# halismai/bpvo

Hardware: AMD Instinct MI355X
Metric: GN iterations/s (1241x376 bit-planes 8ch, 4 levels, Tukey; linearise + solve + update = 1, the reference's _num_fun_evals) (higher is better)
Workload: dtype f32 (+f64 projection/interpolation)

## Files before the change

bpvo_amd/csrc/kernels_frame.hip:

```cpp
#include <algorithm>
#include <cstdlib>

#include "frame_common.h"

namespace bpvo_hip {

__device__ __forceinline__ const FrameJob& level_job(const FrameJob* jobs, unsigned z, int nframes, int job_pitch)
{
  const unsigned lvl = z / (unsigned) nframes;
  return jobs[(size_t) lvl * job_pitch + (z - lvl * (unsigned) nframes)];
}

__global__ __launch_bounds__(256) void ingest_kernel(const FrameJob* jobs, const uint8_t* images, const float* disps, size_t npix, int skip_odd_disp)
{
  const FrameJob& j = jobs[blockIdx.z];
  const uint8_t* __restrict__ si = images + (size_t) blockIdx.z * npix;
  const float* __restrict__ sd = disps + (size_t) (skip_odd_disp == 2 ? blockIdx.z / 2 : blockIdx.z) * npix;
  uint8_t* __restrict__ di = const_cast<uint8_t*>(j.img.get());
  float* __restrict__ dd = const_cast<float*>(j.disp.get());
  const size_t t = (size_t) blockIdx.x * 256 + threadIdx.x, stride = (size_t) gridDim.x * 256;
  const bool w4 = (npix % 4 == 0) && (((uintptr_t) si | (uintptr_t) di) % 4 == 0);
  if(w4) {
    const uint32_t* s4 = reinterpret_cast<const uint32_t*>(si);
    uint32_t* d4 = reinterpret_cast<uint32_t*>(di);
    for(size_t k = t; k < npix / 4; k += stride) d4[k] = s4[k];
  } else {
    for(size_t k = t; k < npix; k += stride) di[k] = si[k];
  }
  if(skip_odd_disp && (blockIdx.z & 1)) return;
  const bool f4 = (npix % 4 == 0) && (((uintptr_t) sd | (uintptr_t) dd) % 16 == 0);
  if(f4) {
    const float4* s4 = reinterpret_cast<const float4*>(sd);
    float4* d4 = reinterpret_cast<float4*>(dd);
    for(size_t k = t; k < npix / 4; k += stride) d4[k] = load_stream(s4 + k);
  } else {
    for(size_t k = t; k < npix; k += stride) dd[k] = sd[k];
  }
}

constexpr int PDT_W = 64, PDT_H = 16;
constexpr int PDS_W = 2 * PDT_W + 3, PDS_H = 2 * PDT_H + 3;
constexpr int PDS_DW = (PDS_W + 3 + 3) / 4;
constexpr int PDS_PITCH = 4 * (PDS_DW + 2);
constexpr int PD_STACK = 4;
constexpr int PD_NPRE = (PDS_H * PDS_DW + 255) / 256;
__global__ __launch_bounds__(256) void pyrdown_u8_lds_kernel(const FrameJob* src_jobs, const FrameJob* dst_jobs)
{
  __shared__ __attribute__((aligned(16))) uint8_t s_src[PDS_H][PDS_PITCH];
  __shared__ __attribute__((aligned(8))) uint16_t s_h[PDS_H][PDT_W];
  __shared__ int s_off[PDS_H];
  const FrameJob& sj = src_jobs[blockIdx.z];
  const FrameJob& dj = dst_jobs[blockIdx.z];
  const int sw = sj.cols, sh = sj.rows, dw = dj.cols, dh = dj.rows;
  const int dx0 = blockIdx.x * PDT_W;
  const int lane = threadIdx.x & 63, wave = threadIdx.x >> 6;
  const uint8_t* __restrict__ s = sj.img;
  uint8_t* __restrict__ const d = const_cast<uint8_t*>(dj.img.get());
  const int c_first = 2 * dx0 - 2;
  const bool fast = c_first >= 3 && c_first + PDS_W + 3 <= sw;
  auto row_ptr = [&](int dy0, int r) { return s + (size_t) reflect101(min(2 * dy0 - 2 + r, sh + 1), sh) * sw + c_first; };
  uint32_t pre[PD_NPRE];
  auto prefetch = [&](int dy0) {
#pragma unroll
    for(int k = 0; k < PD_NPRE; ++k) {
      const int i = min((int) threadIdx.x + k * 256, PDS_H * PDS_DW - 1);
      const int r = i / PDS_DW, l = i - r * PDS_DW;
      const uintptr_t a = reinterpret_cast<uintptr_t>(row_ptr(dy0, r));
      const unsigned ll = min((unsigned) l, ((unsigned) (a & 3u) + PDS_W - 1) / 4u);
      pre[k] = *reinterpret_cast<const uint32_t*>(a - (a & 3u) + 4u * ll);
    }
  };
  const int dy_first = blockIdx.y * (PDT_H * PD_STACK);
  if(fast) prefetch(dy_first);
  for(int t = 0; t < PD_STACK; ++t) {
    const int dy0 = dy_first + t * PDT_H;
    if(dy0 >= dh) break;
    if(fast) {
#pragma unroll
      for(int k = 0; k < PD_NPRE; ++k) {
        const int i = (int) threadIdx.x + k * 256;
        if(i < PDS_H * PDS_DW) { const int r = i / PDS_DW, l = i - r * PDS_DW; reinterpret_cast<uint32_t*>(&s_src[r][0])[l] = pre[k]; }
      }
      if(t + 1 < PD_STACK && dy0 + PDT_H < dh) prefetch(dy0 + PDT_H);
    } else {
      for(int r = wave; r < PDS_H; r += 4) {
        const uint8_t* row = s + (size_t) reflect101(min(2 * dy0 - 2 + r, sh + 1), sh) * sw;
#pragma unroll
        for(int c0 = 0; c0 < PDS_W; c0 += 64) {
          const int c = c0 + lane;
          if(c < PDS_W) s_src[r][c] = row[reflect101(min(c_first + c, sw + 1), sw)];
        }
      }
    }
    if(threadIdx.x < PDS_H) s_off[threadIdx.x] = fast ? (int) (reinterpret_cast<uintptr_t>(row_ptr(dy0, threadIdx.x)) & 3u) : 0;
    __syncthreads();
    for(int idx = threadIdx.x; idx < PDS_H * (PDT_W / 4); idx += 256) {
      const int r = idx >> 4, xq = idx & 15;
      const uint2* q = reinterpret_cast<const uint2*>(&s_src[r][8 * xq]);
      const uint2 lo = q[0], hi = q[1];
      const unsigned off = (unsigned) s_off[r];
      const unsigned d0 = __builtin_amdgcn_alignbyte(lo.y, lo.x, off), d1 = __builtin_amdgcn_alignbyte(hi.x, lo.y, off),
                     d2 = __builtin_amdgcn_alignbyte(hi.y, hi.x, off);
      const unsigned kW = 0x04060401u;
      const unsigned h0 = __builtin_amdgcn_udot4(d0, kW, d1 & 0xffu, false);
      const unsigned h1 = __builtin_amdgcn_udot4(__builtin_amdgcn_alignbyte(d1, d0, 2), kW, (d1 >> 16) & 0xffu, false);
      const unsigned h2 = __builtin_amdgcn_udot4(d1, kW, d2 & 0xffu, false);
      const unsigned h3 = __builtin_amdgcn_udot4(__builtin_amdgcn_alignbyte(d2, d1, 2), kW, (d2 >> 16) & 0xffu, false);
      *reinterpret_cast<uint2*>(&s_h[r][4 * xq]) = make_uint2(h0 | (h1 << 16), h2 | (h3 << 16));
    }
    __syncthreads();
    const int ty = threadIdx.x >> 4, xq = threadIdx.x & 15;
    const int y = dy0 + ty, x = dx0 + 4 * xq;
    if(y < dh && x < dw) {
      unsigned v[4];
      uint2 tt[5];
#pragma unroll
      for(int k = 0; k < 5; ++k) tt[k] = *reinterpret_cast<const uint2*>(&s_h[2 * ty + k][4 * xq]);
#pragma unroll
      for(int e = 0; e < 4; ++e) {
        unsigned a[5];
#pragma unroll
        for(int k = 0; k < 5; ++k) { const unsigned w = (e < 2) ? tt[k].x : tt[k].y; a[k] = (e & 1) ? (w >> 16) : (w & 0xffffu); }
        v[e] = (a[0] + 4u * a[1] + 6u * a[2] + 4u * a[3] + a[4] + 128u) >> 8;
      }
      uint8_t* o = d + (size_t) y * dw + x;
      if(x + 3 < dw) {
        typedef uint32_t __attribute__((aligned(1))) u32_unaligned;
        *reinterpret_cast<u32_unaligned*>(o) = v[0] | (v[1] << 8) | (v[2] << 16) | (v[3] << 24);
      } else {
        for(int e = 0; e < 4 && x + e < dw; ++e) o[e] = (uint8_t) v[e];
      }
    }
    __syncthreads();
  }
}

constexpr int PA_T = 8;
constexpr int pa_edge(int steps) { return steps == 0 ? PA_T : 2 * pa_edge(steps - 1) + 3; }
template <int NL>
__global__ __launch_bounds__(256) void pyramid_levels_kernel(const FrameJob* jobs , int job_pitch)
{
  constexpr int E0 = pa_edge(NL), E1 = pa_edge(NL - 1);
  __shared__ uint8_t s_a[E0 * E0];
  __shared__ uint8_t s_b[E1 * E1];
  __shared__ uint16_t s_h[E0 * E1];
  int W[NL + 1], H[NL + 1], xlo[NL + 1], xhi[NL + 1], ylo[NL + 1], yhi[NL + 1];
#pragma unroll
  for(int k = 0; k <= NL; ++k) { const FrameJob& j = jobs[(size_t) k * job_pitch + blockIdx.z]; W[k] = j.cols; H[k] = j.rows; }
  xlo[NL] = blockIdx.x * PA_T; xhi[NL] = min(xlo[NL] + PA_T, W[NL]) - 1;
  ylo[NL] = blockIdx.y * PA_T; yhi[NL] = min(ylo[NL] + PA_T, H[NL]) - 1;
#pragma unroll
  for(int k = NL - 1; k >= 0; --k) {
    xlo[k] = max(0, 2 * xlo[k + 1] - 2); xhi[k] = min(W[k] - 1, 2 * xhi[k + 1] + 2);
    ylo[k] = max(0, 2 * ylo[k + 1] - 2); yhi[k] = min(H[k] - 1, 2 * yhi[k + 1] + 2);
  }
  const int tid = threadIdx.x;
  {
    const uint8_t* __restrict__ src = jobs[blockIdx.z].img;
    const int nx = xhi[0] - xlo[0] + 1, ny = yhi[0] - ylo[0] + 1;
    for(int i = tid; i < nx * ny; i += 256) {
      const int r = i / nx, c = i - r * nx;
      s_a[r * E0 + c] = src[(size_t) (ylo[0] + r) * W[0] + xlo[0] + c];
    }
  }
  __syncthreads();
  uint8_t* cur = s_a;
  uint8_t* nxt = s_b;
  int pc = E0, pn = E1;
#pragma unroll
  for(int k = 0; k < NL; ++k) {
    const int snx = xhi[k] - xlo[k] + 1, sny = yhi[k] - ylo[k] + 1;
    const int dnx = xhi[k + 1] - xlo[k + 1] + 1, dny = yhi[k + 1] - ylo[k + 1] + 1;
    (void) snx;
    for(int i = tid; i < sny * dnx; i += 256) {
      const int r = i / dnx, c = i - r * dnx;
      const int x2 = 2 * (xlo[k + 1] + c);
      const uint8_t* row = cur + r * pc - xlo[k];
      const unsigned a0 = row[reflect101(x2 - 2, W[k])], a1 = row[reflect101(x2 - 1, W[k])], a2 = row[x2], a3 = row[reflect101(x2 + 1, W[k])],
                     a4 = row[reflect101(x2 + 2, W[k])];
      s_h[r * E1 + c] = (uint16_t) (a0 + 4u * a1 + 6u * a2 + 4u * a3 + a4);
    }
    __syncthreads();
    const int sh = NL - (k + 1);
    const int ox0 = (blockIdx.x * PA_T) << sh, ox1 = min(((blockIdx.x + 1) * PA_T) << sh, W[k + 1]);
    const int oy0 = (blockIdx.y * PA_T) << sh, oy1 = min(((blockIdx.y + 1) * PA_T) << sh, H[k + 1]);
    uint8_t* __restrict__ dst = const_cast<uint8_t*>(jobs[(size_t) (k + 1) * job_pitch + blockIdx.z].img.get());
    for(int i = tid; i < dny * dnx; i += 256) {
      const int r = i / dnx, c = i - r * dnx;
      const int y = ylo[k + 1] + r, x = xlo[k + 1] + c, y2 = 2 * y;
      const uint16_t* col = s_h + c - ylo[k] * E1;
      const unsigned b0 = col[reflect101(y2 - 2, H[k]) * E1], b1 = col[reflect101(y2 - 1, H[k]) * E1], b2 = col[y2 * E1],
                     b3 = col[reflect101(y2 + 1, H[k]) * E1], b4 = col[reflect101(y2 + 2, H[k]) * E1];
      const uint8_t v = (uint8_t) ((b0 + 4u * b1 + 6u * b2 + 4u * b3 + b4 + 128u) >> 8);
      nxt[r * pn + c] = v;
      if(x >= ox0 && x < ox1 && y >= oy0 && y < oy1) dst[(size_t) y * W[k + 1] + x] = v;
    }
    __syncthreads();
    { uint8_t* t = cur; cur = nxt; nxt = t; }
    { const int t = pc; pc = pn; pn = t; }
  }
}
void launch_pyramid_levels(hipStream_t s, const FrameJob* src_row, int job_pitch, int steps, int dW, int dR, int nframes)
{
  const dim3 grid((dW + PA_T - 1) / PA_T, (dR + PA_T - 1) / PA_T, nframes);
  if(steps == 3) hipLaunchKernelGGL(pyramid_levels_kernel<3>, grid, dim3(256), 0, s, src_row, job_pitch);
  else if(steps == 2) hipLaunchKernelGGL(pyramid_levels_kernel<2>, grid, dim3(256), 0, s, src_row, job_pitch);
  else hipLaunchKernelGGL(pyramid_levels_kernel<1>, grid, dim3(256), 0, s, src_row, job_pitch);
}

__global__ __launch_bounds__(256) void intensity_kernel(const FrameJob* jobs, int nframes, int job_pitch)
{
  const FrameJob& j = level_job(jobs, blockIdx.z, nframes, job_pitch);
  const int n = j.rows * j.cols;
  const int i = (blockIdx.x * 256 + threadIdx.x) * 4;
  if(i >= n) return;
  if(i + 3 < n && ((uintptr_t) (j.img + i) & 3) == 0) {
    const uchar4 v = *reinterpret_cast<const uchar4*>(j.img + i);
    *reinterpret_cast<float4*>(j.desc + i) = make_float4((float) v.x, (float) v.y, (float) v.z, (float) v.w);
  } else {
    for(int k = i; k < n && k < i + 4; ++k) j.desc[k] = (float) j.img[k];
  }
}

constexpr int ROWS_PER_THREAD = 4;
constexpr int CENSUS_ROWS = 8;
__global__ __launch_bounds__(256) void census_kernel(const FrameJob* jobs)
{
  const FrameJob& j = jobs[blockIdx.z];
  const int x = blockIdx.x * 64 + (threadIdx.x & 63);
  const int y0 = (blockIdx.y * 4 + (threadIdx.x >> 6)) * CENSUS_ROWS;
  const int W = j.cols, R = j.rows;
  if(x >= W || y0 >= R) return;
  const bool xin = x > 0 && x < W - 1;
  const int xm = max(x - 1, 0), xp = min(x + 1, W - 1);
  uint8_t w[CENSUS_ROWS + 2][3];
#pragma unroll
  for(int k = 0; k < CENSUS_ROWS + 2; ++k) {
    const uint8_t* p = j.img + (size_t) min(max(y0 - 1 + k, 0), R - 1) * W;
    w[k][0] = p[xm]; w[k][1] = p[x]; w[k][2] = p[xp];
  }
#pragma unroll
  for(int k = 0; k < CENSUS_ROWS; ++k) {
    const int y = y0 + k;
    if(y < R) {
      uint8_t out = 0;
      if(xin && y > 0 && y < R - 1) {
        const uint8_t ctr = w[k + 1][1];
        out = (uint8_t) (((w[k][0] >= ctr) << 0) | ((w[k][1] >= ctr) << 1) | ((w[k][2] >= ctr) << 2) | ((w[k + 1][0] >= ctr) << 3) |
                         ((w[k + 1][2] >= ctr) << 4) | ((w[k + 2][0] >= ctr) << 5) | ((w[k + 2][1] >= ctr) << 6) | ((w[k + 2][2] >= ctr) << 7));
      }
      j.cen[(size_t) y * W + x] = out;
    }
  }
}

constexpr int CB_TW = 64, CB_TH = 4;
__global__ __launch_bounds__(256) void census_blur_kernel(const FrameJob* jobs, int kc, int ks, int nframes, int job_pitch)
{
  __shared__ uint8_t s_src[(CB_TH + 4) * (CB_TW + 4)];
  __shared__ int s_tmp[(CB_TH + 4) * (CB_TW + 2)];
  __shared__ uint8_t s_b[(CB_TH + 2) * (CB_TW + 2)];
  const FrameJob& j = level_job(jobs, blockIdx.z, nframes, job_pitch);
  const int W = j.cols, R = j.rows;
  const int x0 = blockIdx.x * CB_TW, y0 = blockIdx.y * CB_TH;
  if(x0 >= W || y0 >= R) return;
  const int tid = threadIdx.x;
  for(int i = tid; i < (CB_TH + 4) * (CB_TW + 4); i += 256) {
    const int ly = i / (CB_TW + 4), lx = i - ly * (CB_TW + 4);
    const int gy = reflect101(min(y0 + ly - 2, R + 1), R), gx = reflect101(min(x0 + lx - 2, W + 1), W);
    s_src[i] = j.img[(size_t) gy * W + gx];
  }
  __syncthreads();
  for(int i = tid; i < (CB_TH + 4) * (CB_TW + 2); i += 256) {
    const int ly = i / (CB_TW + 2), lx = i - ly * (CB_TW + 2);
    const uint8_t* p = s_src + ly * (CB_TW + 4) + lx + 1;
    s_tmp[i] = (int) p[0] * kc + ((int) p[-1] + (int) p[1]) * ks;
  }
  __syncthreads();
  for(int i = tid; i < (CB_TH + 2) * (CB_TW + 2); i += 256) {
    const int ly = i / (CB_TW + 2), lx = i - ly * (CB_TW + 2);
    const int* t = s_tmp + (ly + 1) * (CB_TW + 2) + lx;
    const int v = (t[0] * kc + (t[-(CB_TW + 2)] + t[CB_TW + 2]) * ks + (1 << 15)) >> 16;
    s_b[i] = (uint8_t) min(255, max(0, v));
  }
  __syncthreads();
  const int lx = tid & 63, ly = tid >> 6;
  const int x = x0 + lx, y = y0 + ly;
  if(x >= W || y >= R) return;
  uint8_t out = 0;
  if(x > 0 && x < W - 1 && y > 0 && y < R - 1) {
    constexpr int P = CB_TW + 2;
    const uint8_t* p = s_b + (ly + 1) * P + lx + 1;
    const uint8_t c = p[0];
    out = (uint8_t) (((p[-P - 1] >= c) << 0) | ((p[-P] >= c) << 1) | ((p[-P + 1] >= c) << 2) | ((p[-1] >= c) << 3) |
                     ((p[1] >= c) << 4) | ((p[P - 1] >= c) << 5) | ((p[P] >= c) << 6) | ((p[P + 1] >= c) << 7));
  }
  j.cen[(size_t) y * W + x] = out;
}

#ifndef BP_TW_VALUE
#define BP_TW_VALUE 64
#define BP_TH_VALUE 8
#endif
constexpr int BP_TW = BP_TW_VALUE, BP_TH = BP_TH_VALUE, BP_HALO = 2;
constexpr int BP_PLANE = (BP_TH + 2 * BP_HALO) * BP_TW + 8;
__device__ __forceinline__ uint2 spread_planes(unsigned c)
{
  unsigned lo = c & 0xFu, hi = (c >> 4) & 0xFu;
  lo = (lo | (lo << 14)) & 0x00030003u; lo = (lo | (lo << 7)) & 0x01010101u;
  hi = (hi | (hi << 14)) & 0x00030003u; hi = (hi | (hi << 7)) & 0x01010101u;
  return make_uint2(lo, hi);
}

template <bool FROM_IMAGE>
__global__ __launch_bounds__(256) void bitplanes_blur_kernel(const FrameJob* jobs, float k0, float k1, float k2, int stack, int nframes, int job_pitch)
{
  constexpr int CR = BP_TH + 2 * BP_HALO, CC = BP_TW + 2 * BP_HALO;
  constexpr int CW = CC + 4;
  constexpr int IR = CR + 2, IC = CC + 2, IW = IC + 2;
  constexpr int NSRC = FROM_IMAGE ? IR * IC : CR * CC;
  constexpr int NPRE = (NSRC + 255) / 256;
  __shared__ uint2 s_cen[CR * CW];
  __shared__ uint8_t s_img[FROM_IMAGE ? IR * IW : 4];
  __shared__ float s_row[(BP_PLANE + CR * BP_TW) * 4];
  __shared__ float s_lut[18];
  const FrameJob& j = level_job(jobs, blockIdx.z, nframes, job_pitch);
  const int W = j.cols, R = j.rows;
  const int x0 = blockIdx.x * BP_TW;
  if(x0 >= W || (int) blockIdx.y * BP_TH * stack >= R) return;
  const int tid = threadIdx.x;
  const uint8_t* __restrict__ cen = FROM_IMAGE ? j.img : j.cen;
  float* __restrict__ const desc = j.desc;
  float* __restrict__ const ch0 = j.ch0;
  const bool lazy_level = FROM_IMAGE && j.lazy != 0;
  const bool lazy = lazy_level && x0 + BP_TW + 8 <= (W & ~3) && !(x0 == 0 && (W & 3) == 0);
  uint8_t* __restrict__ const cen_out = j.cen;
  if(tid < 18) {
    const float S0 = (float) (tid / 9), A = (float) (tid % 3), B = (float) ((tid / 3) % 3);
    s_lut[tid] = S0 * k0 + A * k1 + B * k2;
  }

  uint8_t pre[NPRE];
  auto prefetch = [&](int y0) {
#pragma unroll
    for(int k = 0; k < NPRE; ++k) {
      const int i = min(tid + k * 256, NSRC - 1);
      if constexpr(FROM_IMAGE) {
        const int ly = i / IC, lx = i - ly * IC;
        const int gy = min(max(y0 + ly - BP_HALO - 1, 0), R - 1), gx = min(max(x0 + lx - BP_HALO - 1, 0), W - 1);
        pre[k] = cen[(size_t) gy * W + gx];
      } else {
        const int ly = i / CC, lx = i - ly * CC;
        const int gy = reflect101(min(y0 + ly - BP_HALO, R + 1), R), gx = reflect101(min(x0 + lx - BP_HALO, W + 1), W);
        pre[k] = cen[(size_t) gy * W + gx];
      }
    }
  };
  auto stage = [&]() {
#pragma unroll
    for(int k = 0; k < NPRE; ++k) {
      const int i = tid + k * 256;
      if constexpr(FROM_IMAGE) {
        if(i < IR * IC) { const int ly = i / IC, lx = i - ly * IC; s_img[ly * IW + lx] = pre[k]; }
      } else {
        if(i < CR * CC) { const int ly = i / CC, lx = i - ly * CC; s_cen[ly * CW + lx] = spread_planes(pre[k]); }
      }
    }
  };
  const int ybase = blockIdx.y * BP_TH * stack;
  prefetch(ybase);
  stage();
  __syncthreads();
  for(int t = 0; t < stack; ++t) {
    const int y0 = ybase + t * BP_TH;
    if(y0 >= R) break;
    if constexpr(FROM_IMAGE) {
      for(int i = tid; i < CR * CC; i += 256) {
        const int ly = i / CC, lx = i - ly * CC;
        const int gy = reflect101(min(y0 + ly - BP_HALO, R + 1), R), gx = reflect101(min(x0 + lx - BP_HALO, W + 1), W);
        uint8_t out = 0;
        if(gx > 0 && gx < W - 1 && gy > 0 && gy < R - 1) {
          const uint8_t* p = s_img + (gy - (y0 - BP_HALO - 1)) * IW + (gx - (x0 - BP_HALO - 1));
          const uint8_t c = p[0];
          out = (uint8_t) (((p[-IW - 1] >= c) << 0) | ((p[-IW] >= c) << 1) | ((p[-IW + 1] >= c) << 2) | ((p[-1] >= c) << 3) |
                           ((p[1] >= c) << 4) | ((p[IW - 1] >= c) << 5) | ((p[IW] >= c) << 6) | ((p[IW + 1] >= c) << 7));
        }
        s_cen[ly * CW + lx] = spread_planes(out);
        if(lazy_level && ly >= BP_HALO && ly < BP_HALO + BP_TH && lx >= BP_HALO && lx < BP_HALO + BP_TW && y0 + ly - BP_HALO < R && x0 + lx - BP_HALO < W)
          cen_out[(size_t) (y0 + ly - BP_HALO) * W + (x0 + lx - BP_HALO)] = out;
      }
      __syncthreads();
    }
    const bool more = t + 1 < stack && y0 + BP_TH < R;
    if(more) prefetch(y0 + BP_TH);

    if(lazy) {
      for(int i = tid; i < CR * BP_TW; i += 256) {
        const int ly = i / BP_TW, lx = i - ly * BP_TW;
        const uint2* c = s_cen + ly * CW + lx;
        const unsigned ilo = (c[1].x + c[3].x) + 3u * (c[0].x + c[4].x) + 9u * c[2].x;
        s_row[i] = s_lut[ilo & 0xffu];
      }
      __syncthreads();
      if(more) stage();
      for(int i = tid; i < BP_TH * BP_TW; i += 256) {
        const int ly = i / BP_TW, lx = i - ly * BP_TW;
        const int gx = x0 + lx, gy = y0 + ly;
        if(gx >= W || gy >= R) continue;
        const float* Th = s_row + ly * BP_TW + lx;
        constexpr int pitch = BP_TW;
        float o = k0 * Th[2 * pitch]; o += k1 * (Th[3 * pitch] + Th[pitch]); o += k2 * (Th[4 * pitch] + Th[0]);
        ch0[(size_t) gy * W + gx] = o;
      }
      __syncthreads();
      continue;
    }
    for(int i = tid; i < CR * BP_TW; i += 256) {
      const int ly = i / BP_TW, lx = i - ly * BP_TW;
      const uint2* c = s_cen + ly * CW + lx;
      const uint2 cm2 = c[0], cm1 = c[1], c0 = c[2], cp1 = c[3], cp2 = c[4];
      const unsigned ilo = (cm1.x + cp1.x) + 3u * (cm2.x + cp2.x) + 9u * c0.x;
      const unsigned ihi = (cm1.y + cp1.y) + 3u * (cm2.y + cp2.y) + 9u * c0.y;
      float tt[8];
#pragma unroll
      for(int b = 0; b < 4; ++b) {
        tt[b] = s_lut[(ilo >> (8 * b)) & 0xffu];
        tt[4 + b] = s_lut[(ihi >> (8 * b)) & 0xffu];
      }
      float4* o = reinterpret_cast<float4*>(s_row);
      o[i] = make_float4(tt[0], tt[1], tt[2], tt[3]);
      o[BP_PLANE + i] = make_float4(tt[4], tt[5], tt[6], tt[7]);
    }
    __syncthreads();
    if(more) stage();

    for(int u = tid; u < 2 * BP_TH * BP_TW; u += 256) {
      const int i = u >> 1, h = u & 1;
      const int ly = i / BP_TW, lx = i - ly * BP_TW;
      const int gx = x0 + lx, gy = y0 + ly;
      if(gx >= W || gy >= R) continue;
      const float4* Th = reinterpret_cast<const float4*>(s_row) + h * BP_PLANE + ly * BP_TW + lx;
      constexpr int pitch = BP_TW;
      const float4 Tm2 = Th[0], Tm1 = Th[pitch], T0 = Th[2 * pitch], Tp1 = Th[3 * pitch], Tp2 = Th[4 * pitch];
      float4 o4;
      o4.x = k0 * T0.x; o4.x += k1 * (Tp1.x + Tm1.x); o4.x += k2 * (Tp2.x + Tm2.x);
      o4.y = k0 * T0.y; o4.y += k1 * (Tp1.y + Tm1.y); o4.y += k2 * (Tp2.y + Tm2.y);
      o4.z = k0 * T0.z; o4.z += k1 * (Tp1.z + Tm1.z); o4.z += k2 * (Tp2.z + Tm2.z);
      o4.w = k0 * T0.w; o4.w += k1 * (Tp1.w + Tm1.w); o4.w += k2 * (Tp2.w + Tm2.w);
      store_stream(reinterpret_cast<float4*>(desc + ((size_t) gy * W + gx) * 8) + h, o4);
      if(h == 0 && ch0) ch0[(size_t) gy * W + gx] = o4.x;
    }
    __syncthreads();
  }
}

__global__ __launch_bounds__(256) void bitplanes_noblur_kernel(const FrameJob* jobs)
{
  const FrameJob& j = jobs[blockIdx.z];
  const int n = j.rows * j.cols;
  const int i = blockIdx.x * 256 + threadIdx.x;
  if(i >= n) return;
  const unsigned c = j.cen[i];
  float4* d = reinterpret_cast<float4*>(j.desc + (size_t) i * 8);
  if(j.ch0) j.ch0[i] = (float) (c & 1u);
  d[0] = make_float4((float) (c & 1u), (float) ((c >> 1) & 1u), (float) ((c >> 2) & 1u), (float) ((c >> 3) & 1u));
  d[1] = make_float4((float) ((c >> 4) & 1u), (float) ((c >> 5) & 1u), (float) ((c >> 6) & 1u), (float) ((c >> 7) & 1u));
}

template <int C>
__device__ __forceinline__ float grad_abs(const float* __restrict__ I, size_t p, int W, int c)
{
  const float Ix = fabsf(I[(p - 1) * C + c] - I[(p + 1) * C + c]);
  const float Iy = fabsf(I[(p - W) * C + c] - I[(p + W) * C + c]);
  return Ix + Iy;
}
template <int C>
__device__ __forceinline__ float grad_tail(const float* __restrict__ I, size_t p, int W, int c)
{
  return fabsf(I[(p + 1) * C + c] - I[(p - 1) * C + c]) + fabsf(I[(p + W) * C + c] + I[(p - W) * C + c]);
}

template <int C>
__global__ __launch_bounds__(256) void saliency_kernel(const FrameJob* jobs)
{
  const FrameJob& j = jobs[blockIdx.z];
  const int W = j.cols, R = j.rows;
  const int x = blockIdx.x * 64 + (threadIdx.x & 63);
  const int y0 = (blockIdx.y * 4 + (threadIdx.x >> 6)) * ROWS_PER_THREAD;
  if(x >= W || y0 >= R) return;
  const float* __restrict__ I = j.desc;
  const int n = W & ~3;
#pragma unroll
  for(int k = 0; k < ROWS_PER_THREAD; ++k) {
    const int y = min(y0 + k, R - 1);
    float S = 0.0f;
    if(y >= 1 && y <= R - 2 && x != W - 1) {
      const size_t row = (size_t) y * W;
      if(x >= n) {
        S = grad_tail<C>(I, row + x, W, 0);
        for(int c = 1; c < C; ++c) S += grad_tail<C>(I, row + x, W, c);
      } else if(C == 1) {
        S = grad_abs<C>(I, row + x, W, 0);
      } else if(x >= 4) {
        if(C == 8 && j.ch0) S = grad_abs<1>(j.ch0, row + x, W, 0);
        else S = grad_abs<C>(I, row + x, W, 0);
      } else {
        const int xs = n - 4 + x;
        const float S0 = (xs == W - 1) ? 0.0f : grad_abs<C>(I, row + xs, W, 0);
        S = S0 + grad_abs<C>(I, row + xs, W, C - 1);
      }
    }
    j.sal[(size_t) y * W + x] = S;
  }
}

__device__ __forceinline__ bool is_local_max(const float* __restrict__ S, int W, int radius, int y, int x)
{
  if(radius <= 0) return true;
  const float* p = S + (size_t) y * W + x;
  const float v = p[0];
  if(radius == 1) {
    float a[4], b[4], c[4];
#pragma unroll
    for(int k = 0; k < 4; ++k) { a[k] = p[k - 1 - W]; b[k] = p[k - 1]; c[k] = p[k - 1 + W]; }
    bool ok = true;
#pragma unroll
    for(int k = 0; k < 4; ++k) {
      if(k != 1) ok = ok & (v > b[k]);
      ok = ok & (v > a[k]) & (v > c[k]);
    }
    return ok;
  }
  for(int r = -radius; r <= radius; ++r)
    for(int c = -radius; c <= radius; ++c)
      if(!(r == 0 && c == 0) && p[r * W + c] >= v) return false;
  return true;
}

#ifndef SEL_PX_VALUE
#define SEL_PX_VALUE 4
#endif
constexpr int SEL_PX = SEL_PX_VALUE;
constexpr int SEL_BLOCK_PX = 256 * SEL_PX;
constexpr int SEL_GROUP = 256 / SEL_PX;
__global__ __launch_bounds__(256) void select_flag_kernel(const FrameJob* jobs, float min_saliency, float min_disp,
                                                          float max_disp, int border)
{
  const FrameJob& j = jobs[blockIdx.z];
  const int W = j.cols, R = j.rows;
  const int npix = W * R;
  const int p0 = blockIdx.x * SEL_BLOCK_PX + threadIdx.x * SEL_PX;
  const float* __restrict__ S = j.sal;
  bool f[SEL_PX];
#pragma unroll
  for(int e = 0; e < SEL_PX; ++e) f[e] = false;
  if(p0 < npix) {
    const int y0 = p0 / W, x0 = p0 - y0 * W;
    const bool one_row = x0 + SEL_PX <= W && p0 + SEL_PX <= npix;
    const bool inner = one_row && j.nms_radius == 1 && y0 >= border && y0 < R - border - 1 && x0 >= border && x0 + SEL_PX - 1 < W - border - 1;
    if(inner) {
      float a[SEL_PX + 3], b[SEL_PX + 3], c[SEL_PX + 3];
      const float* q = S + (size_t) y0 * W + x0 - 1;
#pragma unroll
      for(int k = 0; k < SEL_PX + 3; ++k) { a[k] = q[k - W]; b[k] = q[k]; c[k] = q[k + W]; }
#pragma unroll
      for(int e = 0; e < SEL_PX; ++e) {
        const float v = b[e + 1];
        bool ok = v >= min_saliency;
#pragma unroll
        for(int k = 0; k < 4; ++k) {
          if(k != 1) ok = ok & (v > b[e + k]);
          ok = ok & (v > a[e + k]) & (v > c[e + k]);
        }
        f[e] = ok;
      }
    } else {
#pragma unroll
      for(int e = 0; e < SEL_PX; ++e) {
        const int p = p0 + e;
        if(p < npix) {
          const int y = p / W, x = p - y * W;
          if(y >= border && y < R - border - 1 && x >= border && x < W - border - 1)
            f[e] = S[p] >= min_saliency && is_local_max(S, W, j.nms_radius, y, x);
        }
      }
    }
#pragma unroll
    for(int e = 0; e < SEL_PX; ++e) {
      if(!f[e]) continue;
      const int p = p0 + e;
      const int y = p / W, x = p - y * W;
      const float d = j.disp[(size_t) (1 << j.level) * ((size_t) y * j.disp_cols + x)];
      f[e] = (d >= min_disp && d <= max_disp);
    }
    if(p0 + SEL_PX <= npix) {
#pragma unroll
      for(int e = 0; e < SEL_PX; e += 4)
        *reinterpret_cast<uchar4*>(j.flag + p0 + e) = make_uchar4(f[e], f[e + 1], f[e + 2], f[e + 3]);
    } else {
      for(int e = 0; e < SEL_PX && p0 + e < npix; ++e) j.flag[p0 + e] = f[e] ? 1 : 0;
    }
  }
  int cnt = 0;
#pragma unroll
  for(int e = 0; e < SEL_PX; ++e) cnt += (int) f[e];
#pragma unroll
  for(int o = SEL_GROUP / 2; o >= 1; o >>= 1) cnt += __shfl_xor(cnt, o);
  const int chunk = p0 / 256;
  if((threadIdx.x & (SEL_GROUP - 1)) == 0 && chunk * 256 < npix) j.blk_count[chunk] = cnt;
}

__global__ __launch_bounds__(1024) void select_scan_kernel(const FrameJob* jobs)
{
  const FrameJob& j = jobs[blockIdx.x];
  const int nblk = (j.rows * j.cols + 255) / 256;
  __shared__ int s_wave[16];
  __shared__ int s_carry;
  if(threadIdx.x == 0) s_carry = 0;
  __syncthreads();
  const int lane = threadIdx.x & 63, wave = threadIdx.x >> 6;
  for(int base = 0; base < nblk; base += 1024) {
    const int i = base + threadIdx.x;
    const int v = (i < nblk) ? j.blk_count[i] : 0;
    int incl = v;
#pragma unroll
    for(int o = 1; o < 64; o <<= 1) {
      const int t = __shfl_up(incl, o);
      if(lane >= o) incl += t;
    }
    if(lane == 63) s_wave[wave] = incl;
    __syncthreads();
    int woff = 0;
    for(int w = 0; w < wave; ++w) woff += s_wave[w];
    const int carry = s_carry;
    if(i < nblk) j.blk_count[i] = carry + woff + incl - v;
    __syncthreads();
    if(threadIdx.x == 1023) s_carry = carry + woff + incl;
    __syncthreads();
  }
  if(threadIdx.x == 0) {
    int total = s_carry;
    if(total > j.cap) total = j.cap;
    *j.n_out = total & ~15;
  }
}

__global__ __launch_bounds__(256) void select_write_kernel(const FrameJob* jobs)
{
  const FrameJob& j = jobs[blockIdx.z];
  const int W = j.cols;
  const int npix = W * j.rows;
  const int p0 = blockIdx.x * SEL_BLOCK_PX + threadIdx.x * SEL_PX;
  const int wave_p0 = blockIdx.x * SEL_BLOCK_PX + (threadIdx.x & ~63) * SEL_PX;
  if(wave_p0 >= npix) return;
  const int chunk = p0 / 256;
  unsigned char fe[SEL_PX];
#pragma unroll
  for(int e = 0; e < SEL_PX; ++e) fe[e] = 0;
  if(p0 + SEL_PX <= npix) {
#pragma unroll
    for(int e = 0; e < SEL_PX; e += 4) {
      const uchar4 v = *reinterpret_cast<const uchar4*>(j.flag + p0 + e);
      fe[e] = v.x; fe[e + 1] = v.y; fe[e + 2] = v.z; fe[e + 3] = v.w;
    }
  } else {
    for(int e = 0; e < SEL_PX && p0 + e < npix; ++e) fe[e] = j.flag[p0 + e];
  }
  int mine = 0;
#pragma unroll
  for(int e = 0; e < SEL_PX; ++e) mine += (int) fe[e];
  const int gl = threadIdx.x & (SEL_GROUP - 1);
  int incl = mine;
#pragma unroll
  for(int o = 1; o < SEL_GROUP; o <<= 1) {
    const int t = __shfl_up(incl, o);
    if(gl >= o) incl += t;
  }
  if(!mine) return;
  int rank = j.blk_count[chunk] + incl - mine;
  const int N = *j.n_out;
  const float fx = j.K[0], fy = j.K[4], cx = j.K[2], cy = j.K[5];
  const float Bf = j.b * fx;
#pragma unroll
  for(int e = 0; e < SEL_PX; ++e) {
    if(!fe[e]) continue;
    const int r = rank++;
    if(r >= N) break;
    const int p = p0 + e;
    const int y = p / W, x = p - y * W;
    const float d = j.disp[(size_t) (1 << j.level) * ((size_t) y * j.disp_cols + x)];
    const float Z = (float) ((double) Bf * (1.0 / (double) d));
    const float X = ((float) x - cx) * Z * (1.0f / fx);
    const float Y = ((float) y - cy) * Z * (1.0f / fy);
    j.pts[r] = j.dspace ? make_float4((float) x - cx, (float) y - cy, d, 1.0f) : make_float4(X, Y, Z, 1.0f);
    j.inds[r] = p;
  }
}

constexpr int ST_W = 64, ST_H = 32, ST_ROWS_PER_WAVE = ST_H / 4;
constexpr int ST_CH_ROWS = ST_H + 4, ST_CH_COLS = ST_W + 5, ST_CH_PITCH = 72;
constexpr int ST_S_ROWS = ST_H + 2, ST_S_COLS = ST_W + 3, ST_S_PITCH = 68;

template <int C>
__device__ __forceinline__ float saliency_generic(const FrameJob& j, int x, int y)
{
  const int W = j.cols, R = j.rows, n = W & ~3;
  if(!(y >= 1 && y <= R - 2 && x != W - 1)) return 0.0f;
  const float* __restrict__ I = j.desc;
  const size_t row = (size_t) y * W;
  if(x >= n) {
    float S = grad_tail<C>(I, row + x, W, 0);
    for(int c = 1; c < C; ++c) S += grad_tail<C>(I, row + x, W, c);
    return S;
  }
  if(C == 1 || x >= 4) return grad_abs<C>(I, row + x, W, 0);
  const int xs = n - 4 + x;
  const float S0 = (xs == W - 1) ? 0.0f : grad_abs<C>(I, row + xs, W, 0);
  return S0 + grad_abs<C>(I, row + xs, W, C - 1);
}

template <int C>
__global__ __launch_bounds__(256) void saliency_select_tile_kernel(const FrameJob* jobs, float min_saliency, float min_disp, float max_disp, int border, int nframes, int job_pitch)
{
  __shared__ float s_ch[ST_CH_ROWS][ST_CH_PITCH];
  __shared__ float s_sal[ST_S_ROWS][ST_S_PITCH];
  const FrameJob& j = level_job(jobs, blockIdx.z, nframes, job_pitch);
  const int W = j.cols, R = j.rows, n = W & ~3;
  const int x0 = blockIdx.x * ST_W, y0 = blockIdx.y * ST_H;
  if(x0 >= W || y0 >= R) return;
  const int lane = threadIdx.x & 63, wave = threadIdx.x >> 6;
  const bool compact = C == 8 && j.ch0;
  const float* __restrict__ ch = compact ? j.ch0.get() : j.desc.get();
  const int CS = compact ? 1 : C;
  for(int i = threadIdx.x; i < ST_CH_ROWS * ST_CH_PITCH; i += 256) {
    const int r = i / ST_CH_PITCH, cc = i - r * ST_CH_PITCH;
    if(cc < ST_CH_COLS) {
      const int y = min(max(y0 - 2 + r, 0), R - 1), xx = min(max(x0 - 2 + cc, 0), W - 1);
      s_ch[r][cc] = ch[((size_t) y * W + xx) * CS];
    }
  }
  __syncthreads();
  for(int i = threadIdx.x; i < ST_S_ROWS * ST_S_PITCH; i += 256) {
    const int r = i / ST_S_PITCH, cc = i - r * ST_S_PITCH;
    if(cc >= ST_S_COLS) continue;
    const int y = y0 - 1 + r, xx = x0 - 1 + cc;
    float S = fabsf(s_ch[r + 1][cc] - s_ch[r + 1][cc + 2]) + fabsf(s_ch[r][cc + 1] - s_ch[r + 2][cc + 1]);
    const bool inside = xx >= 0 && xx < W && y >= 0 && y < R;
    if(!(xx >= 4 && xx < n && xx != W - 1 && y >= 1 && y <= R - 2)) S = (inside && (xx < 4 || xx >= n)) ? saliency_generic<C>(j, xx, y) : 0.0f;
    s_sal[r][cc] = S;
  }
  __syncthreads();
  const int x = x0 + lane, c = lane + 1;
  const int radius = j.nms_radius;
// ... 719 lines not shown
```

Baseline: 1.246 million.

## Keep vertical blur column in registers instead of shared-memory row buffer

Result: faster. 1.264 million (median of 6 runs) (+1.4%).

```diff
diff --git a/bpvo_amd/csrc/kernels_frame.hip b/bpvo_amd/csrc/kernels_frame.hip
--- a/bpvo_amd/csrc/kernels_frame.hip
+++ b/bpvo_amd/csrc/kernels_frame.hip
@@ -300,10 +300,9 @@
 
 #ifndef BP_TW_VALUE
 #define BP_TW_VALUE 64
-#define BP_TH_VALUE 8
+#define BP_TH_VALUE 16
 #endif
 constexpr int BP_TW = BP_TW_VALUE, BP_TH = BP_TH_VALUE, BP_HALO = 2;
-constexpr int BP_PLANE = (BP_TH + 2 * BP_HALO) * BP_TW + 8;
 __device__ __forceinline__ uint2 spread_planes(unsigned c)
 {
   unsigned lo = c & 0xFu, hi = (c >> 4) & 0xFu;
@@ -322,7 +321,7 @@
   constexpr int NPRE = (NSRC + 255) / 256;
   __shared__ uint2 s_cen[CR * CW];
   __shared__ uint8_t s_img[FROM_IMAGE ? IR * IW : 4];
-  __shared__ float s_row[(BP_PLANE + CR * BP_TW) * 4];
+  __shared__ float s_row[CR * BP_TW];
   __shared__ float s_lut[18];
   const FrameJob& j = level_job(jobs, blockIdx.z, nframes, job_pitch);
   const int W = j.cols, R = j.rows;
@@ -415,40 +414,30 @@
       __syncthreads();
       continue;
     }
-    for(int i = tid; i < CR * BP_TW; i += 256) {
-      const int ly = i / BP_TW, lx = i - ly * BP_TW;
-      const uint2* c = s_cen + ly * CW + lx;
-      const uint2 cm2 = c[0], cm1 = c[1], c0 = c[2], cp1 = c[3], cp2 = c[4];
-      const unsigned ilo = (cm1.x + cp1.x) + 3u * (cm2.x + cp2.x) + 9u * c0.x;
-      const unsigned ihi = (cm1.y + cp1.y) + 3u * (cm2.y + cp2.y) + 9u * c0.y;
-      float tt[8];
-#pragma unroll
-      for(int b = 0; b < 4; ++b) {
-        tt[b] = s_lut[(ilo >> (8 * b)) & 0xffu];
-        tt[4 + b] = s_lut[(ihi >> (8 * b)) & 0xffu];
-      }
-      float4* o = reinterpret_cast<float4*>(s_row);
-      o[i] = make_float4(tt[0], tt[1], tt[2], tt[3]);
-      o[BP_PLANE + i] = make_float4(tt[4], tt[5], tt[6], tt[7]);
-    }
-    __syncthreads();
-    if(more) stage();
-
-    for(int u = tid; u < 2 * BP_TH * BP_TW; u += 256) {
-      const int i = u >> 1, h = u & 1;
-      const int ly = i / BP_TW, lx = i - ly * BP_TW;
-      const int gx = x0 + lx, gy = y0 + ly;
-      if(gx >= W || gy >= R) continue;
-      const float4* Th = reinterpret_cast<const float4*>(s_row) + h * BP_PLANE + ly * BP_TW + lx;
-      constexpr int pitch = BP_TW;
-      const float4 Tm2 = Th[0], Tm1 = Th[pitch], T0 = Th[2 * pitch], Tp1 = Th[3 * pitch], Tp2 = Th[4 * pitch];
-      float4 o4;
-      o4.x = k0 * T0.x; o4.x += k1 * (Tp1.x + Tm1.x); o4.x += k2 * (Tp2.x + Tm2.x);
-      o4.y = k0 * T0.y; o4.y += k1 * (Tp1.y + Tm1.y); o4.y += k2 * (Tp2.y + Tm2.y);
-      o4.z = k0 * T0.z; o4.z += k1 * (Tp1.z + Tm1.z); o4.z += k2 * (Tp2.z + Tm2.z);
-      o4.w = k0 * T0.w; o4.w += k1 * (Tp1.w + Tm1.w); o4.w += k2 * (Tp2.w + Tm2.w);
-      store_stream(reinterpret_cast<float4*>(desc + ((size_t) gy * W + gx) * 8) + h, o4);
-      if(h == 0 && ch0) ch0[(size_t) gy * W + gx] = o4.x;
+    constexpr int RPL = BP_TH / 2, TRL = RPL + 2 * BP_HALO;
+    static_assert(2 * BP_TW * 2 == 256 && BP_TH % 2 == 0, "one lane pair per column, two row groups");
+    const int h = tid & 1, lx = (tid >> 1) & (BP_TW - 1), ly0 = (tid >> 7) * RPL;
+    const int gx = x0 + lx;
+    float4 T[TRL];
+#pragma unroll
+    for(int r = 0; r < TRL; ++r) {
+      const unsigned* c = reinterpret_cast<const unsigned*>(s_cen + (ly0 + r) * CW + lx) + h;
+      const unsigned idx = (c[2] + c[6]) + 3u * (c[0] + c[8]) + 9u * c[4];
+      T[r] = make_float4(s_lut[idx & 0xffu], s_lut[(idx >> 8) & 0xffu], s_lut[(idx >> 16) & 0xffu], s_lut[idx >> 24]);
+      if constexpr(FROM_IMAGE) { if(r == 2 * BP_HALO && more) stage(); }
+      else if(r == TRL - 1) { __syncthreads(); if(more) stage(); }
+      if(r < 2 * BP_HALO) continue;
+      const int k = r - 2 * BP_HALO, gy = y0 + ly0 + k;
+      if(gx < W && gy < R) {
+        const float4 Tm2 = T[k], Tm1 = T[k + 1], T0 = T[k + 2], Tp1 = T[k + 3], Tp2 = T[k + 4];
+        float4 o4;
+        o4.x = k0 * T0.x; o4.x += k1 * (Tp1.x + Tm1.x); o4.x += k2 * (Tp2.x + Tm2.x);
+        o4.y = k0 * T0.y; o4.y += k1 * (Tp1.y + Tm1.y); o4.y += k2 * (Tp2.y + Tm2.y);
+        o4.z = k0 * T0.z; o4.z += k1 * (Tp1.z + Tm1.z); o4.z += k2 * (Tp2.z + Tm2.z);
+        o4.w = k0 * T0.w; o4.w += k1 * (Tp1.w + Tm1.w); o4.w += k2 * (Tp2.w + Tm2.w);
+        store_stream(reinterpret_cast<float4*>(desc + ((size_t) gy * W + gx) * 8) + h, o4);
+        if(h == 0 && ch0) ch0[(size_t) gy * W + gx] = o4.x;
+      }
     }
     __syncthreads();
   }
```
